# crowsonkb/k-diffusion

Measured on NVIDIA H100. Metric: images/sec (256x256, Heun 50-step), higher is better.
Workload: dtype bf16

## Files before the change

k-diffusion_b200/csrc/tc_common.cuh:

```cuda
#pragma once
#include <cuda.h>

#include "common.cuh"

namespace kdb {
namespace tc {

__device__ __forceinline__ uint32_t smem_u32(const void* p) { return (uint32_t)__cvta_generic_to_shared(p); }

__device__ __forceinline__ void pdl_wait() { asm volatile("griddepcontrol.wait;" ::: "memory"); }
__device__ __forceinline__ void pdl_launch_dependents() { asm volatile("griddepcontrol.launch_dependents;" ::: "memory"); }

__device__ __forceinline__ void mbar_init(uint64_t* bar, uint32_t count) {
  asm volatile("mbarrier.init.shared::cta.b64 [%0], %1;" ::"r"(smem_u32(bar)), "r"(count));
}
__device__ __forceinline__ void fence_barrier_init() { asm volatile("fence.mbarrier_init.release.cluster;" ::: "memory"); }
__device__ __forceinline__ void fence_proxy_async() { asm volatile("fence.proxy.async.shared::cta;" ::: "memory"); }

__device__ __forceinline__ void mbar_arrive_expect_tx(uint64_t* bar, uint32_t bytes) {
  asm volatile("mbarrier.arrive.expect_tx.shared::cta.b64 _, [%0], %1;" ::"r"(smem_u32(bar)), "r"(bytes) : "memory");
}
__device__ __forceinline__ void mbar_arrive(uint64_t* bar) {
  asm volatile("mbarrier.arrive.shared::cta.b64 _, [%0];" ::"r"(smem_u32(bar)) : "memory");
}
__device__ __forceinline__ bool mbar_try_wait(uint64_t* bar, uint32_t parity) {
  uint32_t ok;
  asm volatile(
      "{\n\t.reg .pred p;\n\t"
      "mbarrier.try_wait.parity.shared::cta.b64 p, [%1], %2, %3;\n\t"
      "selp.u32 %0, 1, 0, p;\n\t}"
      : "=r"(ok)
      : "r"(smem_u32(bar)), "r"(parity), "r"(200000u)
      : "memory");
  return ok != 0;
}
__device__ __forceinline__ uint64_t globaltimer_ns() {
  uint64_t t;
  asm volatile("mov.u64 %0, %%globaltimer;" : "=l"(t));
  return t;
}
__device__ __forceinline__ void mbar_wait(uint64_t* bar, uint32_t parity) {
  if (mbar_try_wait(bar, parity)) return;
  const uint64_t t0 = globaltimer_ns();
  uint32_t spins = 0;
  while (!mbar_try_wait(bar, parity)) {
    if ((++spins & 63u) == 0 && globaltimer_ns() - t0 > 2000000000ull) {
      printf("libkdb200: mbarrier wait timed out (block %d,%d,%d thread %d parity %u)\n", blockIdx.x, blockIdx.y, blockIdx.z, threadIdx.x, parity);
      __trap();
    }
  }
}

__device__ __forceinline__ void mbar_wait_nocall(uint64_t* bar, uint32_t parity) {
  if (mbar_try_wait(bar, parity)) return;
  const uint64_t t0 = globaltimer_ns();
  uint32_t spins = 0;
  while (!mbar_try_wait(bar, parity))
    if ((++spins & 63u) == 0 && globaltimer_ns() - t0 > 2000000000ull) __trap();
}

__device__ __forceinline__ void tma_prefetch_desc(const CUtensorMap* m) {
  asm volatile("prefetch.tensormap [%0];" ::"l"(reinterpret_cast<uint64_t>(m)) : "memory");
}
__device__ __forceinline__ void tma_load_2d(void* smem_dst, const CUtensorMap* map, uint64_t* bar, int c0, int c1) {
  asm volatile("cp.async.bulk.tensor.2d.shared::cluster.global.mbarrier::complete_tx::bytes [%0], [%1, {%3, %4}], [%2];" ::"r"(
                   smem_u32(smem_dst)),
               "l"(reinterpret_cast<uint64_t>(map)), "r"(smem_u32(bar)), "r"(c0), "r"(c1)
               : "memory");
}
__device__ __forceinline__ void tma_load_3d(void* smem_dst, const CUtensorMap* map, uint64_t* bar, int c0, int c1, int c2) {
  asm volatile("cp.async.bulk.tensor.3d.shared::cluster.global.mbarrier::complete_tx::bytes [%0], [%1, {%3, %4, %5}], [%2];" ::"r"(
                   smem_u32(smem_dst)),
               "l"(reinterpret_cast<uint64_t>(map)), "r"(smem_u32(bar)), "r"(c0), "r"(c1), "r"(c2)
               : "memory");
}
__device__ __forceinline__ void tma_load_4d(void* smem_dst, const CUtensorMap* map, uint64_t* bar, int c0, int c1, int c2, int c3) {
  asm volatile("cp.async.bulk.tensor.4d.shared::cluster.global.mbarrier::complete_tx::bytes [%0], [%1, {%3, %4, %5, %6}], [%2];" ::"r"(
                   smem_u32(smem_dst)),
               "l"(reinterpret_cast<uint64_t>(map)), "r"(smem_u32(bar)), "r"(c0), "r"(c1), "r"(c2), "r"(c3)
               : "memory");
}

__device__ __forceinline__ void tma_load_5d(void* smem_dst, const CUtensorMap* map, uint64_t* bar, int c0, int c1, int c2, int c3, int c4) {
  asm volatile("cp.async.bulk.tensor.5d.shared::cluster.global.mbarrier::complete_tx::bytes [%0], [%1, {%3, %4, %5, %6, %7}], [%2];" ::"r"(
                   smem_u32(smem_dst)),
               "l"(reinterpret_cast<uint64_t>(map)), "r"(smem_u32(bar)), "r"(c0), "r"(c1), "r"(c2), "r"(c3), "r"(c4)
               : "memory");
}
__device__ __forceinline__ void tma_store_4d(const CUtensorMap* map, const void* smem_src, int c0, int c1, int c2, int c3) {
  asm volatile("cp.async.bulk.tensor.4d.global.shared::cta.bulk_group [%0, {%2, %3, %4, %5}], [%1];" ::"l"(reinterpret_cast<uint64_t>(map)),
               "r"(smem_u32(smem_src)), "r"(c0), "r"(c1), "r"(c2), "r"(c3)
               : "memory");
}
__device__ __forceinline__ void tma_store_3d(const CUtensorMap* map, const void* smem_src, int c0, int c1, int c2) {
  asm volatile("cp.async.bulk.tensor.3d.global.shared::cta.bulk_group [%0, {%2, %3, %4}], [%1];" ::"l"(reinterpret_cast<uint64_t>(map)),
               "r"(smem_u32(smem_src)), "r"(c0), "r"(c1), "r"(c2)
               : "memory");
}
__device__ __forceinline__ void tma_store_2d(const CUtensorMap* map, const void* smem_src, int c0, int c1) {
  asm volatile("cp.async.bulk.tensor.2d.global.shared::cta.bulk_group [%0, {%2, %3}], [%1];" ::"l"(reinterpret_cast<uint64_t>(map)),
               "r"(smem_u32(smem_src)), "r"(c0), "r"(c1)
               : "memory");
}
__device__ __forceinline__ void tma_store_commit() { asm volatile("cp.async.bulk.commit_group;" ::: "memory"); }
__device__ __forceinline__ void tma_store_wait_read() { asm volatile("cp.async.bulk.wait_group.read 0;" ::: "memory"); }
__device__ __forceinline__ void named_barrier_sync(int id, int threads) { asm volatile("bar.sync %0, %1;" ::"r"(id), "r"(threads) : "memory"); }
__device__ __forceinline__ void named_barrier_arrive(int id, int threads) { asm volatile("bar.arrive %0, %1;" ::"r"(id), "r"(threads) : "memory"); }

template <uint32_t R> __device__ __forceinline__ void setmaxnreg_dec() { asm volatile("setmaxnreg.dec.sync.aligned.u32 %0;" ::"n"(R)); }
template <uint32_t R> __device__ __forceinline__ void setmaxnreg_inc() { asm volatile("setmaxnreg.inc.sync.aligned.u32 %0;" ::"n"(R)); }

__device__ __forceinline__ uint32_t sw128_offset(int row, int chunk16) {
  return (uint32_t)((row >> 3) * 1024 + (row & 7) * 128 + ((chunk16 ^ (row & 7)) << 4));
}

__device__ __forceinline__ void wg_fence() { asm volatile("wgmma.fence.sync.aligned;" ::: "memory"); }
__device__ __forceinline__ void wg_commit() { asm volatile("wgmma.commit_group.sync.aligned;" ::: "memory"); }
template <int N>
__device__ __forceinline__ void wg_wait() { asm volatile("wgmma.wait_group.sync.aligned %0;" ::"n"(N) : "memory"); }
template <int R>
__device__ __forceinline__ void wg_fence_acc(float (&d)[R]) {
#pragma unroll
  for (int i = 0; i < R; ++i) asm volatile("" : "+f"(d[i])::"memory");
}
template <int R>
__device__ __forceinline__ void wg_fence_acc(uint32_t (&d)[R]) {
#pragma unroll
  for (int i = 0; i < R; ++i) asm volatile("" : "+r"(d[i])::"memory");
}

__device__ __forceinline__ void wgmma_128(float (&d)[64], uint64_t adesc, uint64_t bdesc, uint32_t accumulate) {
  asm volatile(
      "{\n\t.reg .pred p;\n\t"
      "setp.ne.b32 p, %66, 0;\n\t"
      "wgmma.mma_async.sync.aligned.m64n128k16.f32.bf16.bf16 "
      "{%0, %1, %2, %3, %4, %5, %6, %7, %8, %9, %10, %11, %12, %13, %14, %15, %16, %17, %18, %19, %20, %21, %22, %23, %24, %25, %26, %27, %28, %29, %30, %31, %32, %33, %34, %35, %36, %37, %38, %39, %40, %41, %42, %43, %44, %45, %46, %47, %48, %49, %50, %51, %52, %53, %54, %55, %56, %57, %58, %59, %60, %61, %62, %63}, %64, %65, p, 1, 1, 0, 0;\n\t}"
      : "+f"(d[0]), "+f"(d[1]), "+f"(d[2]), "+f"(d[3]), "+f"(d[4]), "+f"(d[5]), "+f"(d[6]), "+f"(d[7]), "+f"(d[8]), "+f"(d[9]), "+f"(d[10]), "+f"(d[11]), "+f"(d[12]), "+f"(d[13]), "+f"(d[14]), "+f"(d[15]), "+f"(d[16]), "+f"(d[17]), "+f"(d[18]), "+f"(d[19]), "+f"(d[20]), "+f"(d[21]), "+f"(d[22]), "+f"(d[23]), "+f"(d[24]), "+f"(d[25]), "+f"(d[26]), "+f"(d[27]), "+f"(d[28]), "+f"(d[29]), "+f"(d[30]), "+f"(d[31]), "+f"(d[32]), "+f"(d[33]), "+f"(d[34]), "+f"(d[35]), "+f"(d[36]), "+f"(d[37]), "+f"(d[38]), "+f"(d[39]), "+f"(d[40]), "+f"(d[41]), "+f"(d[42]), "+f"(d[43]), "+f"(d[44]), "+f"(d[45]), "+f"(d[46]), "+f"(d[47]), "+f"(d[48]), "+f"(d[49]), "+f"(d[50]), "+f"(d[51]), "+f"(d[52]), "+f"(d[53]), "+f"(d[54]), "+f"(d[55]), "+f"(d[56]), "+f"(d[57]), "+f"(d[58]), "+f"(d[59]), "+f"(d[60]), "+f"(d[61]), "+f"(d[62]), "+f"(d[63])
      : "l"(adesc), "l"(bdesc), "r"(accumulate));
}
template <int TB>
__device__ __forceinline__ void wgmma_64(float (&d)[32], uint64_t adesc, uint64_t bdesc, uint32_t accumulate) {
  asm volatile(
      "{\n\t.reg .pred p;\n\t"
      "setp.ne.b32 p, %34, 0;\n\t"
      "wgmma.mma_async.sync.aligned.m64n64k16.f32.bf16.bf16 "
      "{%0, %1, %2, %3, %4, %5, %6, %7, %8, %9, %10, %11, %12, %13, %14, %15, %16, %17, %18, %19, %20, %21, %22, %23, %24, %25, %26, %27, %28, %29, %30, %31}, %32, %33, p, 1, 1, 0, %35;\n\t}"
      : "+f"(d[0]), "+f"(d[1]), "+f"(d[2]), "+f"(d[3]), "+f"(d[4]), "+f"(d[5]), "+f"(d[6]), "+f"(d[7]), "+f"(d[8]), "+f"(d[9]), "+f"(d[10]), "+f"(d[11]), "+f"(d[12]), "+f"(d[13]), "+f"(d[14]), "+f"(d[15]), "+f"(d[16]), "+f"(d[17]), "+f"(d[18]), "+f"(d[19]), "+f"(d[20]), "+f"(d[21]), "+f"(d[22]), "+f"(d[23]), "+f"(d[24]), "+f"(d[25]), "+f"(d[26]), "+f"(d[27]), "+f"(d[28]), "+f"(d[29]), "+f"(d[30]), "+f"(d[31])
      : "l"(adesc), "l"(bdesc), "r"(accumulate), "n"(TB));
}
__device__ __forceinline__ void wgmma_128_rs(float (&d)[64], const uint32_t (&a)[4], uint64_t bdesc, uint32_t accumulate) {
  asm volatile(
      "{\n\t.reg .pred p;\n\t"
      "setp.ne.b32 p, %69, 0;\n\t"
      "wgmma.mma_async.sync.aligned.m64n128k16.f32.bf16.bf16 "
      "{%0, %1, %2, %3, %4, %5, %6, %7, %8, %9, %10, %11, %12, %13, %14, %15, %16, %17, %18, %19, %20, %21, %22, %23, %24, %25, %26, %27, %28, %29, %30, %31, %32, %33, %34, %35, %36, %37, %38, %39, %40, %41, %42, %43, %44, %45, %46, %47, %48, %49, %50, %51, %52, %53, %54, %55, %56, %57, %58, %59, %60, %61, %62, %63}, {%64, %65, %66, %67}, %68, p, 1, 1, 0;\n\t}"
      : "+f"(d[0]), "+f"(d[1]), "+f"(d[2]), "+f"(d[3]), "+f"(d[4]), "+f"(d[5]), "+f"(d[6]), "+f"(d[7]), "+f"(d[8]), "+f"(d[9]), "+f"(d[10]), "+f"(d[11]), "+f"(d[12]), "+f"(d[13]), "+f"(d[14]), "+f"(d[15]), "+f"(d[16]), "+f"(d[17]), "+f"(d[18]), "+f"(d[19]), "+f"(d[20]), "+f"(d[21]), "+f"(d[22]), "+f"(d[23]), "+f"(d[24]), "+f"(d[25]), "+f"(d[26]), "+f"(d[27]), "+f"(d[28]), "+f"(d[29]), "+f"(d[30]), "+f"(d[31]), "+f"(d[32]), "+f"(d[33]), "+f"(d[34]), "+f"(d[35]), "+f"(d[36]), "+f"(d[37]), "+f"(d[38]), "+f"(d[39]), "+f"(d[40]), "+f"(d[41]), "+f"(d[42]), "+f"(d[43]), "+f"(d[44]), "+f"(d[45]), "+f"(d[46]), "+f"(d[47]), "+f"(d[48]), "+f"(d[49]), "+f"(d[50]), "+f"(d[51]), "+f"(d[52]), "+f"(d[53]), "+f"(d[54]), "+f"(d[55]), "+f"(d[56]), "+f"(d[57]), "+f"(d[58]), "+f"(d[59]), "+f"(d[60]), "+f"(d[61]), "+f"(d[62]), "+f"(d[63])
      : "r"(a[0]), "r"(a[1]), "r"(a[2]), "r"(a[3]), "l"(bdesc), "r"(accumulate));
}

template <int TB>
__device__ __forceinline__ void wgmma_64_rs(float (&d)[32], const uint32_t (&a)[4], uint64_t bdesc, uint32_t accumulate) {
  asm volatile(
      "{\n\t.reg .pred p;\n\t"
      "setp.ne.b32 p, %37, 0;\n\t"
      "wgmma.mma_async.sync.aligned.m64n64k16.f32.bf16.bf16 "
      "{%0, %1, %2, %3, %4, %5, %6, %7, %8, %9, %10, %11, %12, %13, %14, %15, %16, %17, %18, %19, %20, %21, %22, %23, %24, %25, %26, %27, %28, %29, %30, %31}, {%32, %33, %34, %35}, %36, p, 1, 1, %38;\n\t}"
      : "+f"(d[0]), "+f"(d[1]), "+f"(d[2]), "+f"(d[3]), "+f"(d[4]), "+f"(d[5]), "+f"(d[6]), "+f"(d[7]), "+f"(d[8]), "+f"(d[9]), "+f"(d[10]), "+f"(d[11]), "+f"(d[12]), "+f"(d[13]), "+f"(d[14]), "+f"(d[15]), "+f"(d[16]), "+f"(d[17]), "+f"(d[18]), "+f"(d[19]), "+f"(d[20]), "+f"(d[21]), "+f"(d[22]), "+f"(d[23]), "+f"(d[24]), "+f"(d[25]), "+f"(d[26]), "+f"(d[27]), "+f"(d[28]), "+f"(d[29]), "+f"(d[30]), "+f"(d[31])
      : "r"(a[0]), "r"(a[1]), "r"(a[2]), "r"(a[3]), "l"(bdesc), "r"(accumulate), "n"(TB));
}

template <int R>
__device__ __forceinline__ void acc_store(float* s, int ld, int row0, const float (&d)[R]) {
  const int t = threadIdx.x & 127;
  const int r = row0 + 16 * (t >> 5) + ((t & 31) >> 2), c = 2 * (t & 3);
#pragma unroll
  for (int j = 0; j < R / 4; ++j) {
    *reinterpret_cast<float2*>(s + (size_t)r * ld + 8 * j + c) = make_float2(d[4 * j], d[4 * j + 1]);
    *reinterpret_cast<float2*>(s + (size_t)(r + 8) * ld + 8 * j + c) = make_float2(d[4 * j + 2], d[4 * j + 3]);
  }
}
__device__ __forceinline__ void acc_ld32(const float* s, int ld, int row, int col0, float (&v)[32]) {
  const float4* src = reinterpret_cast<const float4*>(s + (size_t)row * ld + col0);
#pragma unroll
  for (int i = 0; i < 8; ++i) {
    const float4 q = src[i];
    v[4 * i] = q.x;
// ... 100 lines not shown
```

k-diffusion_b200/csrc/tc_kernels.cu:

```cuda
#include "tc_common.cuh"
#include "tc_kernels.cuh"

namespace kdb {

typedef CUresult (*EncodeTiledFn)(CUtensorMap*, CUtensorMapDataType, cuuint32_t, void*, const cuuint64_t*, const cuuint64_t*,
                                  const cuuint32_t*, const cuuint32_t*, CUtensorMapInterleave, CUtensorMapSwizzle,
                                  CUtensorMapL2promotion, CUtensorMapFloatOOBfill);

static EncodeTiledFn encode_fn() {
  static EncodeTiledFn fn = [] {
    void* p = nullptr;
    cudaDriverEntryPointQueryResult q;
    if (cudaGetDriverEntryPoint("cuTensorMapEncodeTiled", &p, cudaEnableDefault, &q) != cudaSuccess) p = nullptr;
    return reinterpret_cast<EncodeTiledFn>(p);
  }();
  return fn;
}

int make_tmap_bf16(CUtensorMap* out, const void* base, int rank, const uint64_t* dims, const uint64_t* strides_bytes, const uint32_t* box) {
  EncodeTiledFn fn = encode_fn();
  KDB_REQUIRE(fn != nullptr, KDB_ERR_UNSUPPORTED, "cuTensorMapEncodeTiled not available from this driver");
  cuuint64_t gd[5];
  cuuint64_t gs[5];
  cuuint32_t bx[5], es[5];
  for (int i = 0; i < rank; ++i) {
    gd[i] = dims[i];
    bx[i] = box[i];
    es[i] = 1;
    if (i > 0) gs[i - 1] = strides_bytes[i - 1];
  }
  CUresult r = fn(out, CU_TENSOR_MAP_DATA_TYPE_BFLOAT16, (cuuint32_t)rank, const_cast<void*>(base), gd, gs, bx, es,
                  CU_TENSOR_MAP_INTERLEAVE_NONE, CU_TENSOR_MAP_SWIZZLE_128B, CU_TENSOR_MAP_L2_PROMOTION_L2_256B,
                  CU_TENSOR_MAP_FLOAT_OOB_FILL_NONE);
  KDB_REQUIRE(r == CUDA_SUCCESS, KDB_ERR_BAD_ARG, "cuTensorMapEncodeTiled failed with CUresult %d (rank %d, dim0 %llu, box0 %u)", (int)r,
              rank, (unsigned long long)dims[0], box[0]);
  return 0;
}

bool pdl_enabled() {
  static const bool enabled = [] {
    const char* e = getenv("KDB200_NO_PDL");
    return !(e != nullptr && e[0] == '1');
  }();
  return enabled;
}

namespace {

constexpr int BM = 128, BK = 64;
constexpr int A_STAGE_BYTES = BM * BK * 2;
constexpr int SUB_TILE_BYTES = BM * 128;
constexpr int GEMM_THREADS = 384;
constexpr int GEMM_RING_BYTES = 96 * 1024;

enum TcEpi { TCE_STORE = 0, TCE_RESID = 1, TCE_GEGLU = 2, TCE_SPLIT = 3, TCE_QKV = 4, TCE_PATCHOUT = 5 };

struct TcParams {
  bf16* out;
  const bf16* resid;
  const float* fac;
  int64_t M;
  int N, K;
  int hc, wc, Cf;
  const float2* rope;
  const float* qk_scale;
  int C, nh, T;
  float* fout;
  const float* x_in;
  const float* sigma;
  float sd;
  int H, Wimg, th, tw;
  const float* ss_in;
  float* ss_out;
  int a_merge, mwc, mC;
  int box_w, box_h;
};

__device__ __forceinline__ float bf16_round(float v) { return __bfloat162float(__float2bfloat16_rn(v)); }

int tmap_2d(CUtensorMap* t, const void* base, uint64_t inner, uint64_t outer, uint32_t box_inner, uint32_t box_outer) {
  const uint64_t dims[2] = {inner, outer};
  const uint64_t strides[1] = {inner * 2};
  const uint32_t box[2] = {box_inner, box_outer};
  return make_tmap_bf16(t, base, 2, dims, strides, box);
}

int tmap_quad(CUtensorMap* t, const void* base, int C, int wc, uint64_t bhc, int box_w, int box_h) {
  const uint64_t dims[5] = {(uint64_t)C, 2, (uint64_t)wc, 2, bhc};
  const uint64_t strides[4] = {(uint64_t)C * 2, (uint64_t)C * 4, (uint64_t)wc * C * 4, (uint64_t)wc * C * 8};
  const uint32_t box[5] = {64, 1, (uint32_t)box_w, 1, (uint32_t)box_h};
  return make_tmap_bf16(t, base, 5, dims, strides, box);
}

bool quad_box(int wc, int* box_w, int* box_h) {
  if (wc >= BM) {
    if (wc % BM != 0) return false;
    *box_w = BM;
    *box_h = 1;
    return true;
  }
  if (BM % wc != 0) return false;
  *box_w = wc;
  *box_h = BM / wc;
  return true;
}

template <int BN, int EPI> constexpr int out_bytes() {
  return EPI == TCE_GEGLU ? SUB_TILE_BYTES : (EPI == TCE_SPLIT || EPI == TCE_PATCHOUT) ? 0 : (BN / 64) * SUB_TILE_BYTES;
}
template <int BN, int EPI> constexpr size_t gemm_smem() { return 1024 + GEMM_RING_BYTES + BM * BN * 4 + 2 * out_bytes<BN, EPI>() + 128; }

template <int BN> __device__ __forceinline__ int stage_off(int row, int chunk) { return row * BN + ((chunk ^ (row & 7)) << 2); }
template <int BN>
__device__ __forceinline__ void stage_store(float* s, int row0, const float (&d)[BN / 2]) {
  const int t = threadIdx.x & 127;
  const int r = row0 + 16 * (t >> 5) + ((t & 31) >> 2), c = 2 * (t & 3);
#pragma unroll
  for (int j = 0; j < BN / 8; ++j) {
    *reinterpret_cast<float2*>(s + stage_off<BN>(r, 2 * j + (c >> 2)) + (c & 3)) = make_float2(d[4 * j], d[4 * j + 1]);
    *reinterpret_cast<float2*>(s + stage_off<BN>(r + 8, 2 * j + (c >> 2)) + (c & 3)) = make_float2(d[4 * j + 2], d[4 * j + 3]);
  }
}
template <int BN>
__device__ __forceinline__ void stage_ld32(const float* s, int row, int col0, float (&v)[32]) {
#pragma unroll
  for (int i = 0; i < 8; ++i) {
    const float4 q = *reinterpret_cast<const float4*>(s + stage_off<BN>(row, (col0 >> 2) + i));
    v[4 * i] = q.x;
    v[4 * i + 1] = q.y;
    v[4 * i + 2] = q.z;
    v[4 * i + 3] = q.w;
  }
}

template <int BN, int EPI>
__global__ void __launch_bounds__(GEMM_THREADS, 1) gemm_wg_kernel(const __grid_constant__ CUtensorMap tma, const __grid_constant__ CUtensorMap tmb,
                                                                  const __grid_constant__ CUtensorMap tmc, const __grid_constant__ CUtensorMap tmr,
                                                                  const TcParams p) {
  KDB_PDL_TRIGGER();
  extern __shared__ uint8_t smem_raw[];
  constexpr int B_STAGE_BYTES = BN * BK * 2;
  constexpr int STAGE_BYTES = A_STAGE_BYTES + B_STAGE_BYTES;
  constexpr int STAGES = GEMM_RING_BYTES / STAGE_BYTES;
  constexpr int NSUB = BN / 64;
  constexpr bool RES = EPI == TCE_RESID;
  uint8_t* base = reinterpret_cast<uint8_t*>((reinterpret_cast<uintptr_t>(smem_raw) + 1023) & ~(uintptr_t)1023);
  float* sAcc = reinterpret_cast<float*>(base + GEMM_RING_BYTES);
  uint64_t* full = reinterpret_cast<uint64_t*>(base + GEMM_RING_BYTES + BM * BN * 4 + 2 * out_bytes<BN, EPI>());
  uint64_t* empty = full + STAGES;
  uint64_t* resid_full = empty + STAGES;

  const int warp = threadIdx.x >> 5, lane = threadIdx.x & 31;
  const int nkb = p.K / BK;
  const int n_tiles = p.N / BN;
  const int tiles = (int)((p.M + BM - 1) / BM) * n_tiles;
  const int n_local = (int)blockIdx.x < tiles ? (tiles - 1 - (int)blockIdx.x) / (int)gridDim.x + 1 : 0;

  if (threadIdx.x == 0) {
    tc::tma_prefetch_desc(&tma);
    tc::tma_prefetch_desc(&tmb);
    for (int s = 0; s < STAGES; ++s) {
      tc::mbar_init(&full[s], 1);
      tc::mbar_init(&empty[s], 4);
    }
    tc::mbar_init(&resid_full[0], 1);
    tc::mbar_init(&resid_full[1], 1);
    tc::fence_barrier_init();
  }
  __syncthreads();
  tc::pdl_wait();

  if (warp >= 8) {
    tc::setmaxnreg_dec<40>();
    if (warp == 8 && tc::elect_one()) {
      int it = 0;
      for (int i = 0; i < n_local; ++i) {
        const int t = (int)blockIdx.x + i * (int)gridDim.x;
        const int64_t m0 = (int64_t)(t / n_tiles) * BM;
        const int n0 = (t % n_tiles) * BN;
        for (int kb = 0; kb < nkb; ++kb, ++it) {
          const int s = it % STAGES;
          tc::mbar_wait_nocall(&empty[s], ((uint32_t)(it / STAGES) & 1u) ^ 1u);
          tc::mbar_arrive_expect_tx(&full[s], STAGE_BYTES);
          uint8_t* a = base + (size_t)s * STAGE_BYTES;
          if (p.a_merge) {
            const int qd = (kb * BK) / p.mC, e0 = kb * BK - qd * p.mC;
            tc::tma_load_5d(a, &tma, &full[s], e0, qd & 1, p.box_h == 1 ? (int)(m0 % p.mwc) : 0, qd >> 1, (int)(m0 / p.mwc));
          } else {
            tc::tma_load_2d(a, &tma, &full[s], kb * BK, (int)m0);
          }
          tc::tma_load_2d(a + A_STAGE_BYTES, &tmb, &full[s], kb * BK, n0);
        }
      }
    }
    return;
  }
  tc::setmaxnreg_inc<232>();

  const int wg = warp >> 2;
  const int row = threadIdx.x & 127;
  uint8_t* sC = base + GEMM_RING_BYTES + BM * BN * 4 + wg * out_bytes<BN, EPI>();
  const int ebar = 1 + wg;
  for (int i = wg; i < n_local; i += 2) {
    const int t = (int)blockIdx.x + i * (int)gridDim.x;
    const int64_t m0 = (int64_t)(t / n_tiles) * BM;
    const int n0 = (t % n_tiles) * BN;
    if constexpr (RES) {
      if (row == 0) {
        tc::mbar_arrive_expect_tx(&resid_full[wg], NSUB * SUB_TILE_BYTES);
#pragma unroll
        for (int g = 0; g < NSUB; ++g) tc::tma_load_2d(sC + g * SUB_TILE_BYTES, &tmr, &resid_full[wg], n0 + g * 64, (int)m0);
      }
    }

    float acc0[BN / 2], acc1[BN / 2];
#pragma unroll
    for (int k = 0; k < BN / 2; ++k) acc0[k] = acc1[k] = 0.f;
    if (i > 0) tc::named_barrier_sync(3 + wg, 256);
    const int it0 = i * nkb;
    for (int kb = 0; kb < nkb; ++kb) {
      const int s = (it0 + kb) % STAGES;
      tc::mbar_wait_nocall(&full[s], (uint32_t)((it0 + kb) / STAGES) & 1u);
      const uint32_t a_addr = tc::smem_u32(base + (size_t)s * STAGE_BYTES);
      const uint64_t ad0 = tc::smem_desc_k_sw128(a_addr), ad1 = tc::smem_desc_k_sw128(a_addr + 8 * 1024);
      const uint64_t bd = tc::smem_desc_k_sw128(a_addr + A_STAGE_BYTES);
      tc::wg_fence_acc(acc0);
      tc::wg_fence_acc(acc1);
      tc::wg_fence();
#pragma unroll
      for (int k = 0; k < BK / 16; ++k) {
        if constexpr (BN == 128) {
          tc::wgmma_128(acc0, ad0 + 2ull * k, bd + 2ull * k, 1u);
          tc::wgmma_128(acc1, ad1 + 2ull * k, bd + 2ull * k, 1u);
        } else {
          tc::wgmma_64<0>(acc0, ad0 + 2ull * k, bd + 2ull * k, 1u);
          tc::wgmma_64<0>(acc1, ad1 + 2ull * k, bd + 2ull * k, 1u);
        }
      }
      tc::wg_commit();
      tc::wg_wait<1>();
      tc::wg_fence_acc(acc0);
      tc::wg_fence_acc(acc1);
      if (kb > 0 && lane == 0) tc::mbar_arrive(&empty[(it0 + kb - 1) % STAGES]);
    }
    if (i + 1 < n_local) tc::named_barrier_arrive(3 + (wg ^ 1), 256);
    tc::wg_wait<0>();
    tc::wg_fence_acc(acc0);
    tc::wg_fence_acc(acc1);
    if (lane == 0) tc::mbar_arrive(&empty[(it0 + nkb - 1) % STAGES]);
    if (i > 0) tc::named_barrier_sync(5 + wg, 256);
    stage_store<BN>(sAcc, 0, acc0);
    stage_store<BN>(sAcc, 64, acc1);
    tc::named_barrier_sync(ebar, 128);
    const bool pass_acc = i + 1 < n_local;

    const int64_t m = m0 + row;
    float rstd = 1.f;
    if (p.ss_in != nullptr) {
      const float4* sp = reinterpret_cast<const float4*>(p.ss_in + (m < p.M ? m : 0) * SS_PARTS);
      rstd = rsqrtf(tc::rowss_sum(__ldg(sp), __ldg(sp + 1), p.K >> 7) / (float)p.K + 1e-6f);
    }
    if constexpr (EPI == TCE_PATCHOUT) {
      float v[64];
      {
        float t0[32], t1[32];
        stage_ld32<BN>(sAcc, row, 0, t0);
        stage_ld32<BN>(sAcc, row, 32, t1);
#pragma unroll
        for (int k = 0; k < 32; ++k) { v[k] = t0[k]; v[32 + k] = t1[k]; }
      }
      if (pass_acc) tc::named_barrier_arrive(5 + (wg ^ 1), 256);
      if (m < p.M) {
        if (p.ss_in != nullptr) {
#pragma unroll
          for (int k = 0; k < 48; ++k) v[k] *= rstd;
        }
        const int per = p.th * p.tw;
        const int b = (int)(m / per);
        const int r = (int)(m - (int64_t)b * per);
        const int ty = r / p.tw, tx = r - ty * p.tw;
        float c_skip = 0.f, c_out = 1.f, c_in;
        if (p.sd > 0.f) karras_scalings(__ldg(p.sigma + b), p.sd, c_skip, c_out, c_in);
#pragma unroll
        for (int c = 0; c < 3; ++c)
#pragma unroll
          for (int nh = 0; nh < 4; ++nh) {
            const int64_t o = (((int64_t)b * 3 + c) * p.H + (ty * 4 + nh)) * p.Wimg + tx * 4;
            float4 y = make_float4(bf16_round(v[(nh * 4 + 0) * 3 + c]), bf16_round(v[(nh * 4 + 1) * 3 + c]), bf16_round(v[(nh * 4 + 2) * 3 + c]),
                                   bf16_round(v[(nh * 4 + 3) * 3 + c]));
            if (p.sd > 0.f) {
              const float4 xi = __ldg(reinterpret_cast<const float4*>(p.x_in + o));
              y = make_float4(y.x * c_out + xi.x * c_skip, y.y * c_out + xi.y * c_skip, y.z * c_out + xi.z * c_skip, y.w * c_out + xi.w * c_skip);
            }
            *reinterpret_cast<float4*>(p.fout + o) = y;
          }
      }
    } else if constexpr (EPI == TCE_SPLIT) {
      const bool live = m < p.M;
      const float facv = __ldg(p.fac);
      float ss = 0.f;
      int64_t fine = 0;
#pragma unroll 1
      for (int c = 0; c < BN / 32; ++c) {
        float v[32];
        stage_ld32<BN>(sAcc, row, c * 32, v);
        if (c == BN / 32 - 1 && pass_acc) tc::named_barrier_arrive(5 + (wg ^ 1), 256);
        if (!live) continue;
        const int n = n0 + c * 32;
        const int64_t b = m / ((int64_t)p.hc * p.wc);
        const int r = (int)(m - b * p.hc * p.wc);
        const int hy = r / p.wc, wx = r - hy * p.wc;
        const int qd = n / p.Cf, e = n - qd * p.Cf;
        fine = (b * (2 * p.hc) + (2 * hy + (qd >> 1))) * (2 * p.wc) + (2 * wx + (qd & 1));
        const int64_t off = fine * p.Cf + e;
        const uint4* sk = reinterpret_cast<const uint4*>(p.resid + off);
        uint4* dst = reinterpret_cast<uint4*>(p.out + off);
#pragma unroll
        for (int j = 0; j < 4; ++j) {
          const uint4 r4 = sk[j];
          const uint32_t rw[4] = {r4.x, r4.y, r4.z, r4.w};
          uint32_t ow[4];
#pragma unroll
          for (int q = 0; q < 4; ++q) {
            const float lo = __uint_as_float(rw[q] << 16), hi = __uint_as_float(rw[q] & 0xffff0000u);
            const float e0 = v[j * 8 + q * 2], e1 = v[j * 8 + q * 2 + 1];
            const float d0 = e0 - lo, d1 = e1 - hi;
            const float o0 = (facv < 0.5f) ? fmaf(facv, d0, lo) : e0 - d0 * (1.f - facv);
            const float o1 = (facv < 0.5f) ? fmaf(facv, d1, hi) : e1 - d1 * (1.f - facv);
            ss = fmaf(o0, o0, fmaf(o1, o1, ss));
            ow[q] = tc::pack_bf16x2(o0, o1);
          }
          dst[j] = make_uint4(ow[0], ow[1], ow[2], ow[3]);
        }
      }
      if (p.ss_out != nullptr && live) p.ss_out[fine * SS_PARTS + ((n0 % p.Cf) >> 7)] = ss;
    } else {
      if constexpr (RES) tc::mbar_wait_nocall(&resid_full[wg], (uint32_t)(i >> 1) & 1u);
      float ss_acc[4] = {0.f, 0.f, 0.f, 0.f};
#pragma unroll 1
      for (int g = 0; g < NSUB; ++g) {
        float v[64];
        {
          float t0[32], t1[32];
          stage_ld32<BN>(sAcc, row, g * 64, t0);
          stage_ld32<BN>(sAcc, row, g * 64 + 32, t1);
#pragma unroll
          for (int k = 0; k < 32; ++k) { v[k] = t0[k]; v[32 + k] = t1[k]; }
        }
        if (g == NSUB - 1 && pass_acc) tc::named_barrier_arrive(5 + (wg ^ 1), 256);
        if (EPI != TCE_GEGLU && p.ss_in != nullptr) {
          bool apply = true;
          if constexpr (EPI == TCE_QKV) apply = (n0 + g * 64) >= 2 * p.C;
          if (apply) {
#pragma unroll
            for (int k = 0; k < 64; ++k) v[k] *= rstd;
          }
        }
        if constexpr (EPI == TCE_GEGLU) {
          const tc::f32x2 r2 = tc::pk2(rstd, rstd), rh = tc::pk2(0.5f * rstd, 0.5f * rstd);
#pragma unroll
          for (int gg = 0; gg < 4; ++gg) {
            uint32_t o[4];
#pragma unroll
            for (int j = 0; j < 4; ++j) {
              tc::f32x2 val = tc::pk2(v[gg * 16 + 2 * j], v[gg * 16 + 2 * j + 1]);
              tc::f32x2 gate = tc::pk2(v[gg * 16 + 8 + 2 * j], v[gg * 16 + 8 + 2 * j + 1]);
              val = tc::mul2(val, rh);
              if (p.ss_in != nullptr) gate = tc::mul2(gate, r2);
              float o0, o1;
              tc::upk2(tc::geglu2(val, gate), o0, o1);
              o[j] = tc::pack_bf16x2(o0, o1);
            }
            *reinterpret_cast<uint4*>(sC + tc::sw128_offset(row, g * 4 + gg)) = make_uint4(o[0], o[1], o[2], o[3]);
          }
        } else {
          uint8_t* cg = sC + g * SUB_TILE_BYTES;
          if constexpr (RES) {
#pragma unroll
            for (int j = 0; j < 8; ++j) {
              const uint4 r4 = *reinterpret_cast<const uint4*>(cg + tc::sw128_offset(row, j));
              const uint32_t rw[4] = {r4.x, r4.y, r4.z, r4.w};
#pragma unroll
              for (int q = 0; q < 4; ++q) {
                v[j * 8 + q * 2] += __uint_as_float(rw[q] << 16);
                v[j * 8 + q * 2 + 1] += __uint_as_float(rw[q] & 0xffff0000u);
              }
            }
          }
          if constexpr (RES || EPI == TCE_STORE) {
            if (p.ss_out != nullptr) {
#pragma unroll
              for (int k = 0; k < 64; k += 4) {
                ss_acc[0] = fmaf(v[k], v[k], ss_acc[0]);
                ss_acc[1] = fmaf(v[k + 1], v[k + 1], ss_acc[1]);
                ss_acc[2] = fmaf(v[k + 2], v[k + 2], ss_acc[2]);
                ss_acc[3] = fmaf(v[k + 3], v[k + 3], ss_acc[3]);
              }
            }
          }
          if constexpr (EPI == TCE_QKV) {
            const int n = n0 + g * 64;
            const int t3 = n / p.C, head = (n - t3 * p.C) >> 6;
            if (t3 < 2) {
              const int64_t tok = (m < p.M ? m : 0) % p.T;
              const float4* tb = reinterpret_cast<const float4*>(p.rope) + (int64_t)head * 8 * p.T + tok;
              tc::f32x2 P[32];
#pragma unroll
              for (int k = 0; k < 32; ++k) P[k] = tc::pk2(v[2 * k], v[2 * k + 1]);
              tc::f32x2 q0 = tc::mul2(P[0], P[0]), q1 = tc::mul2(P[1], P[1]), q2 = tc::mul2(P[2], P[2]), q3 = tc::mul2(P[3], P[3]);
#pragma unroll
              for (int k = 4; k < 32; k += 4) {
                q0 = tc::fma2(P[k], P[k], q0);
                q1 = tc::fma2(P[k + 1], P[k + 1], q1);
                q2 = tc::fma2(P[k + 2], P[k + 2], q2);
                q3 = tc::fma2(P[k + 3], P[k + 3], q3);
              }
              const float sc = sqrtf(__ldg(p.qk_scale + head)) * rsqrtf(((q0.x + q0.y) + (q1.x + q1.y)) + ((q2.x + q2.y) + (q3.x + q3.y)) + 1e-6f);
              const tc::f32x2 sc2 = tc::pk2(sc, sc);
#pragma unroll
              for (int k = 0; k < 8; ++k) {
                const float4 cs = __ldg(tb + (int64_t)k * p.T);
                const tc::f32x2 C = tc::pk2(cs.x, cs.y), S = tc::pk2(cs.z, cs.w);
                const tc::f32x2 X1 = P[k], X2 = P[8 + k];
                P[k] = tc::mul2(tc::fma2(X2, tc::neg2(S), tc::mul2(X1, C)), sc2);
                P[8 + k] = tc::mul2(tc::fma2(X1, S, tc::mul2(X2, C)), sc2);
              }
#pragma unroll
              for (int k = 16; k < 32; ++k) P[k] = tc::mul2(P[k], sc2);
#pragma unroll
              for (int k = 0; k < 32; ++k) tc::upk2(P[k], v[2 * k], v[2 * k + 1]);
            }
          }
#pragma unroll
          for (int j = 0; j < 8; ++j)
            *reinterpret_cast<uint4*>(cg + tc::sw128_offset(row, j)) =
                make_uint4(tc::pack_bf16x2(v[j * 8 + 0], v[j * 8 + 1]), tc::pack_bf16x2(v[j * 8 + 2], v[j * 8 + 3]),
                           tc::pack_bf16x2(v[j * 8 + 4], v[j * 8 + 5]), tc::pack_bf16x2(v[j * 8 + 6], v[j * 8 + 7]));
        }
      }
      if constexpr (RES || EPI == TCE_STORE) {
        if (p.ss_out != nullptr && m < p.M) p.ss_out[m * SS_PARTS + (n0 >> 7)] = (ss_acc[0] + ss_acc[1]) + (ss_acc[2] + ss_acc[3]);
      }
      tc::fence_proxy_async();
      tc::named_barrier_sync(ebar, 128);
      if (row == 0) {
        if constexpr (EPI == TCE_GEGLU) {
          tc::tma_store_2d(&tmc, sC, n0 / 2, (int)m0);
        } else {
#pragma unroll
          for (int g = 0; g < NSUB; ++g) tc::tma_store_2d(&tmc, sC + g * SUB_TILE_BYTES, n0 + g * 64, (int)m0);
        }
        tc::tma_store_commit();
        tc::tma_store_wait_read();
      }
    }
  }
}


#include "tc_ffn_fused.cuh"
#include "tc_attn_block.cuh"

template <int BN, int EPI>
int launch_tc(const bf16* A, const bf16* W, const TcParams& p, cudaStream_t st) {
  CUtensorMap ta, tb, tcm, tr;
  int rc;
  if (p.a_merge) {
    if ((rc = tmap_quad(&ta, A, p.mC, p.mwc, (uint64_t)p.M / p.mwc, p.box_w, p.box_h))) return rc;
  } else {
    if ((rc = tmap_2d(&ta, A, (uint64_t)p.K, (uint64_t)p.M, BK, BM))) return rc;
  }
  if ((rc = tmap_2d(&tb, W, (uint64_t)p.K, (uint64_t)p.N, BK, BN))) return rc;
  const uint64_t n_out = EPI == TCE_GEGLU ? (uint64_t)p.N / 2 : (uint64_t)p.N;
  if (EPI != TCE_SPLIT && EPI != TCE_PATCHOUT) {
    if ((rc = tmap_2d(&tcm, p.out, n_out, (uint64_t)p.M, 64, BM))) return rc;
  } else {
    tcm = ta;
  }
  if (EPI == TCE_RESID) {
    if ((rc = tmap_2d(&tr, p.resid, (uint64_t)p.N, (uint64_t)p.M, 64, BM))) return rc;
  } else {
    tr = ta;
  }
  constexpr size_t smem = gemm_smem<BN, EPI>();
  static_assert(smem <= 227 * 1024, "GEMM shared memory exceeds the 227 KiB opt-in limit");
  static bool attr_set = false;
  if (!attr_set) {
    KDB_CUDA(cudaFuncSetAttribute(gemm_wg_kernel<BN, EPI>, cudaFuncAttributeMaxDynamicSharedMemorySize, (int)smem));
    attr_set = true;
  }
  const int64_t tiles = ceil_div(p.M, BM) * (p.N / BN);
  KDB_CUDA(launch_pdl(gemm_wg_kernel<BN, EPI>, dim3((unsigned)(tiles < num_sms() ? tiles : num_sms())), dim3(GEMM_THREADS), smem, st, ta, tb, tcm,
                      tr, p));
  KDB_LAUNCH_CHECK(EPI == TCE_PATCHOUT ? F_PATCH_OUT : F_GEMM_TC, st);
  return 0;
}

template <int EPI>
int dispatch_bn(const bf16* A, const bf16* W, const TcParams& p, cudaStream_t st) {
  if (p.N % 128 == 0) return launch_tc<128, EPI>(A, W, p, st);
  return launch_tc<64, EPI>(A, W, p, st);
}

bool shape_ok(int64_t M, int N, int K) {
  return M > 0 && M < (65535LL * BM) && N >= 64 && N % 64 == 0 && K >= 64 && K % 64 == 0;
}

}

namespace {
struct PatchInParams {
  const float* x;
  const float* sigma;
  float sd;
  int64_t M;
  int H, Wimg, th, tw, N;
  float* ss_out;
};

constexpr int PATCH_IN_THREADS = 160;
constexpr int PATCH_IN_LD = 132;
constexpr size_t PATCH_IN_SMEM = 1024 + 2 * A_STAGE_BYTES + (size_t)BM * PATCH_IN_LD * 4 + 2 * SUB_TILE_BYTES + 64;

__global__ void __launch_bounds__(PATCH_IN_THREADS) patch_in_tc_kernel(const __grid_constant__ CUtensorMap tmw, const __grid_constant__ CUtensorMap tmc,
                                                                   const PatchInParams p) {
  KDB_PDL_TRIGGER();
  extern __shared__ uint8_t smem_raw[];
  constexpr int LD = PATCH_IN_LD;
  uint8_t* base = reinterpret_cast<uint8_t*>((reinterpret_cast<uintptr_t>(smem_raw) + 1023) & ~(uintptr_t)1023);
  uint8_t* sA = base;
  uint8_t* sW = base + A_STAGE_BYTES;
  uint8_t* sC = sW + A_STAGE_BYTES;
  float* sAcc = reinterpret_cast<float*>(sC + 2 * SUB_TILE_BYTES);
  uint64_t* w_full = reinterpret_cast<uint64_t*>(sAcc + BM * LD);

  const int warp = threadIdx.x >> 5;
  const int64_t m0 = (int64_t)blockIdx.x * BM;
  const int n0 = blockIdx.y * 128;
  if (threadIdx.x == 0) {
    tc::tma_prefetch_desc(&tmw);
    tc::tma_prefetch_desc(&tmc);
    tc::mbar_init(w_full, 1);
    tc::fence_barrier_init();
  }
  __syncthreads();

  if (warp == 4) {
    if (tc::elect_one()) {
      tc::mbar_arrive_expect_tx(w_full, A_STAGE_BYTES);
      tc::tma_load_2d(sW, &tmw, w_full, 0, n0);
    }
    return;
  }
  const int row = threadIdx.x;
  const int64_t m = m0 + row;
  uint4 chunk[6];
  if (m < p.M) {
    const int per = p.th * p.tw;
    const int b = (int)(m / per);
    const int r = (int)(m - (int64_t)b * per);
    const int ty = r / p.tw, tx = r - ty * p.tw;
    float c_in = 1.f;
    if (p.sd > 0.f) {
      const float sg = __ldg(p.sigma + b);
      c_in = rsqrtf(fmaf(sg, sg, p.sd * p.sd));
// ... 70 lines not shown
  tc::fence_proxy_async();
  tc::named_barrier_sync(1, 128);
  if (threadIdx.x == 0) {
    tc::tma_store_2d(&tmc, sC, n0, (int)m0);
    tc::tma_store_2d(&tmc, sC + SUB_TILE_BYTES, n0 + 64, (int)m0);
    tc::tma_store_commit();
    tc::tma_store_wait_read();
  }
}

__global__ void __launch_bounds__(256) patch_in_weight_kernel(const float* __restrict__ W, bf16* __restrict__ out, int N) {
  for (int i = blockIdx.x * 256 + threadIdx.x; i < N * 64; i += gridDim.x * 256) {
    const int n = i >> 6, k = i & 63;
    float v = 0.f;
    if (k < 48) {
      const int c = k >> 4, nh = (k >> 2) & 3, nw = k & 3;
      v = W[(int64_t)n * 48 + (nh * 4 + nw) * 3 + c];
    }
    out[i] = __float2bfloat16(v);
  }
}

}

static bool g_tc_disabled = [] {
  const char* e = getenv("KDB200_DISABLE_TC");
  return e != nullptr && e[0] == '1';
}();

bool tc_gemm_supported(int64_t M, int N, int K, const GemmEpi& epi) {
  if (g_tc_disabled || !shape_ok(M, N, K)) return false;
  if (epi.ss_in != nullptr && (N % 128 != 0 || K % 128 != 0 || K > 128 * SS_PARTS || (epi.mode != EPI_STORE && epi.mode != EPI_QKV_ROPE) || epi.mC > 0))
    return false;
  if (epi.mC > 0) {
    int bw, bh;
    if (epi.mode != EPI_STORE || N % 128 != 0 || epi.mC % 64 != 0 || K != 4 * epi.mC || M % epi.mwc != 0 || !quad_box(epi.mwc, &bw, &bh)) return false;
  }
  if (epi.mode == EPI_SPLIT_LERP) return epi.C % 32 == 0 && N == 4 * epi.C;
  if (epi.mode == EPI_QKV_ROPE) return N == 3 * epi.C && epi.C % 64 == 0 && epi.nh * 64 == epi.C && epi.rope != nullptr;
  return epi.mode == EPI_STORE || epi.mode == EPI_RESID;
}

bool tc_gemm_emits_rowss(int64_t M, int N, int K, const GemmEpi& epi) {
  if (!tc_gemm_supported(M, N, K, epi)) return false;
  if (N % 128 != 0) return false;
  if (epi.mode == EPI_RESID || epi.mode == EPI_STORE) return N <= 128 * SS_PARTS;
  if (epi.mode == EPI_SPLIT_LERP) return epi.C % 128 == 0 && epi.C <= 128 * SS_PARTS;
  return false;
}

int launch_gemm_tc(const bf16* A, const bf16* W, bf16* C, int64_t M, int N, int K, const GemmEpi& epi, cudaStream_t st) {
  KDB_REQUIRE(shape_ok(M, N, K), KDB_ERR_BAD_SHAPE, "gemm_tc: unsupported shape M=%lld N=%d K=%d", (long long)M, N, K);
  KDB_REQUIRE((reinterpret_cast<uintptr_t>(A) & 15) == 0 && (reinterpret_cast<uintptr_t>(W) & 15) == 0 && (reinterpret_cast<uintptr_t>(C) & 15) == 0,
              KDB_ERR_BAD_ARG, "gemm_tc: operands must be 16-byte aligned");
  TcParams p{};
  p.out = C;
  p.M = M;
  p.N = N;
  p.K = K;
  p.ss_in = epi.ss_in;
  p.ss_out = epi.ss_out;
  KDB_REQUIRE(epi.ss_in == nullptr || tc_gemm_supported(M, N, K, epi), KDB_ERR_UNSUPPORTED, "gemm_tc: fused-norm geometry not supported");
  KDB_REQUIRE(epi.ss_out == nullptr || tc_gemm_emits_rowss(M, N, K, epi), KDB_ERR_UNSUPPORTED, "gemm_tc: this shape cannot emit row statistics");
  if (epi.mC > 0) {
    KDB_REQUIRE(tc_gemm_supported(M, N, K, epi), KDB_ERR_UNSUPPORTED, "gemm_tc: token-merge geometry not supported");
    p.a_merge = 1;
    p.mC = epi.mC;
    p.mwc = epi.mwc;
    quad_box(epi.mwc, &p.box_w, &p.box_h);
    return launch_tc<128, TCE_STORE>(A, W, p, st);
  }
  switch (epi.mode) {
    case EPI_STORE:
      return dispatch_bn<TCE_STORE>(A, W, p, st);
    case EPI_RESID:
      p.resid = static_cast<const bf16*>(epi.resid);
      return dispatch_bn<TCE_RESID>(A, W, p, st);
    case EPI_SPLIT_LERP:
      p.resid = static_cast<const bf16*>(epi.resid);
      p.fac = epi.fac;
      p.hc = epi.hc;
      p.wc = epi.wc;
      p.Cf = epi.C;
      return dispatch_bn<TCE_SPLIT>(A, W, p, st);
    case EPI_QKV_ROPE:
      p.rope = epi.rope;
      p.qk_scale = epi.qk_scale;
      p.C = epi.C;
      p.nh = epi.nh;
      p.T = epi.T_tokens;
      return dispatch_bn<TCE_QKV>(A, W, p, st);
    default:
      KDB_REQUIRE(false, KDB_ERR_BAD_ARG, "gemm_tc: bad epilogue");
  }
}

bool tc_patch_out_supported(int C0, int Cout, int ph, int pw, int Wimg) {
  return !g_tc_disabled && C0 % 64 == 0 && Cout == 3 && ph == 4 && pw == 4 && Wimg % 4 == 0;
}

int launch_patch_out_tc(const bf16* xn, const bf16* W_pad, const float* x_in, const float* sigma, float sigma_data, float* out, int B, int H,
                        int Wimg, int C0, cudaStream_t st, const float* ss_in) {
  KDB_REQUIRE(ss_in == nullptr || (C0 % 128 == 0 && C0 <= 128 * SS_PARTS), KDB_ERR_UNSUPPORTED, "patch_out_tc: fused norm needs C0 %% 128 == 0");
  KDB_REQUIRE((reinterpret_cast<uintptr_t>(out) & 15) == 0 && (sigma_data <= 0.f || (reinterpret_cast<uintptr_t>(x_in) & 15) == 0), KDB_ERR_BAD_ARG,
              "patch_out_tc: x and out must be 16-byte aligned (float4 epilogue)");
  TcParams p{};
  p.ss_in = ss_in;
  p.M = (int64_t)B * (H / 4) * (Wimg / 4);
  p.N = 64;
  p.K = C0;
  p.fout = out;
  p.x_in = x_in;
  p.sigma = sigma;
  p.sd = sigma_data;
  p.H = H;
  p.Wimg = Wimg;
  p.th = H / 4;
  p.tw = Wimg / 4;
  KDB_REQUIRE(shape_ok(p.M, 64, C0), KDB_ERR_BAD_SHAPE, "patch_out_tc: unsupported shape");
  return launch_tc<64, TCE_PATCHOUT>(xn, W_pad, p, st);
}

bool tc_patch_in_supported(int Cin, int ph, int pw, int C0, int Wimg) {
  return !g_tc_disabled && Cin == 3 && ph == 4 && pw == 4 && C0 % 128 == 0 && C0 <= 128 * SS_PARTS && Wimg % 4 == 0;
}

int prepare_patch_in_weight(const float* W, bf16* out, int C0, cudaStream_t st) {
  patch_in_weight_kernel<<<(unsigned)ceil_div((int64_t)C0 * 64, 256), 256, 0, st>>>(W, out, C0);
  KDB_LAUNCH_CHECK(F_CONVERT, st);
  return 0;
}

int launch_patch_in_tc(const float* x, const float* sigma, float sigma_data, const bf16* W_perm, bf16* out, int B, int H, int Wimg, int C0,
                       float* ss_out, cudaStream_t st) {
  PatchInParams p{};
  p.x = x;
  p.sigma = sigma;
  p.sd = sigma_data;
  p.H = H;
  p.Wimg = Wimg;
  p.th = H / 4;
  p.tw = Wimg / 4;
  p.M = (int64_t)B * p.th * p.tw;
  p.N = C0;
  p.ss_out = ss_out;
  KDB_REQUIRE((reinterpret_cast<uintptr_t>(x) & 15) == 0, KDB_ERR_BAD_ARG, "patch_in_tc: input must be 16-byte aligned");
  CUtensorMap tw, tcm;
  int rc;
  if ((rc = tmap_2d(&tw, W_perm, 64, (uint64_t)C0, 64, 128))) return rc;
  if ((rc = tmap_2d(&tcm, out, (uint64_t)C0, (uint64_t)p.M, 64, BM))) return rc;
  const size_t smem = PATCH_IN_SMEM;
  static bool attr_set = false;
  if (!attr_set) {
    KDB_CUDA(cudaFuncSetAttribute(patch_in_tc_kernel, cudaFuncAttributeMaxDynamicSharedMemorySize, (int)smem));
    attr_set = true;
  }
  patch_in_tc_kernel<<<dim3((unsigned)ceil_div(p.M, BM), (unsigned)(C0 / 128)), PATCH_IN_THREADS, smem, st>>>(tw, tcm, p);
  KDB_LAUNCH_CHECK(F_PATCH_IN, st);
  return 0;
}

bool tc_gemm_geglu_supported(int64_t M, int N2, int K, bool fused_norm) {
  if (fused_norm && (K % 128 != 0 || K > 128 * SS_PARTS)) return false;
  return !g_tc_disabled && shape_ok(M, N2, K) && N2 % 128 == 0;
}

// ... 95 lines not shown
```

Baseline: 125.5.

## Use TMA preload and TMA store for split-lerp GEMM epilogue

Adds a TCE_SPLIT_TMA epilogue variant for the token-split/lerp GEMM. It prefetches the skip/residual tile into shared memory with a 5D TMA load in the quad layout, does the lerp in swizzled smem, and writes the result back with 5D TMA stores. This replaces the per-thread scattered global loads and stores of the old split epilogue. It is dispatched only when C is a multiple of 64 and the tile fits a quad box; otherwise the old path is kept. It also adds unused multicast and cluster helpers.

```diff
diff --git a/k-diffusion_b200/csrc/tc_common.cuh b/k-diffusion_b200/csrc/tc_common.cuh
--- a/k-diffusion_b200/csrc/tc_common.cuh
+++ b/k-diffusion_b200/csrc/tc_common.cuh
@@ -87,6 +87,11 @@
                "l"(reinterpret_cast<uint64_t>(map)), "r"(smem_u32(bar)), "r"(c0), "r"(c1), "r"(c2), "r"(c3), "r"(c4)
                : "memory");
 }
+__device__ __forceinline__ void tma_store_5d(const CUtensorMap* map, const void* smem_src, int c0, int c1, int c2, int c3, int c4) {
+  asm volatile("cp.async.bulk.tensor.5d.global.shared::cta.bulk_group [%0, {%2, %3, %4, %5, %6}], [%1];" ::"l"(reinterpret_cast<uint64_t>(map)),
+               "r"(smem_u32(smem_src)), "r"(c0), "r"(c1), "r"(c2), "r"(c3), "r"(c4)
+               : "memory");
+}
 __device__ __forceinline__ void tma_store_4d(const CUtensorMap* map, const void* smem_src, int c0, int c1, int c2, int c3) {
   asm volatile("cp.async.bulk.tensor.4d.global.shared::cta.bulk_group [%0, {%2, %3, %4, %5}], [%1];" ::"l"(reinterpret_cast<uint64_t>(map)),
                "r"(smem_u32(smem_src)), "r"(c0), "r"(c1), "r"(c2), "r"(c3)
@@ -102,6 +107,31 @@
                "r"(smem_u32(smem_src)), "r"(c0), "r"(c1)
                : "memory");
 }
+__device__ __forceinline__ void tma_load_2d_mc(void* smem_dst, const CUtensorMap* map, uint64_t* bar, int c0, int c1, uint16_t cta_mask) {
+  asm volatile(
+      "cp.async.bulk.tensor.2d.shared::cluster.global.mbarrier::complete_tx::bytes.multicast::cluster [%0], [%1, {%3, %4}], [%2], %5;" ::"r"(
+          smem_u32(smem_dst)),
+      "l"(reinterpret_cast<uint64_t>(map)), "r"(smem_u32(bar)), "r"(c0), "r"(c1), "h"(cta_mask)
+      : "memory");
+}
+
+__device__ __forceinline__ uint32_t cluster_ctarank() {
+  uint32_t r;
+  asm volatile("mov.u32 %0, %%cluster_ctarank;" : "=r"(r));
+  return r;
+}
+__device__ __forceinline__ void cluster_sync() {
+  asm volatile("barrier.cluster.arrive.release.aligned;\n\tbarrier.cluster.wait.acquire.aligned;" ::: "memory");
+}
+__device__ __forceinline__ void mbar_arrive_cluster(uint64_t* bar, uint32_t cta) {
+  asm volatile(
+      "{\n\t.reg .b32 ra;\n\t"
+      "mapa.shared::cluster.u32 ra, %0, %1;\n\t"
+      "mbarrier.arrive.shared::cluster.b64 _, [ra];\n\t}" ::"r"(smem_u32(bar)),
+      "r"(cta)
+      : "memory");
+}
+
 __device__ __forceinline__ void tma_store_commit() { asm volatile("cp.async.bulk.commit_group;" ::: "memory"); }
 __device__ __forceinline__ void tma_store_wait_read() { asm volatile("cp.async.bulk.wait_group.read 0;" ::: "memory"); }
 __device__ __forceinline__ void named_barrier_sync(int id, int threads) { asm volatile("bar.sync %0, %1;" ::"r"(id), "r"(threads) : "memory"); }
diff --git a/k-diffusion_b200/csrc/tc_kernels.cu b/k-diffusion_b200/csrc/tc_kernels.cu
--- a/k-diffusion_b200/csrc/tc_kernels.cu
+++ b/k-diffusion_b200/csrc/tc_kernels.cu
@@ -53,7 +53,7 @@
 constexpr int GEMM_THREADS = 384;
 constexpr int GEMM_RING_BYTES = 96 * 1024;
 
-enum TcEpi { TCE_STORE = 0, TCE_RESID = 1, TCE_GEGLU = 2, TCE_SPLIT = 3, TCE_QKV = 4, TCE_PATCHOUT = 5 };
+enum TcEpi { TCE_STORE = 0, TCE_RESID = 1, TCE_GEGLU = 2, TCE_SPLIT = 3, TCE_QKV = 4, TCE_PATCHOUT = 5, TCE_SPLIT_TMA = 6 };
 
 struct TcParams {
   bf16* out;
@@ -144,6 +144,7 @@
   constexpr int STAGES = GEMM_RING_BYTES / STAGE_BYTES;
   constexpr int NSUB = BN / 64;
   constexpr bool RES = EPI == TCE_RESID;
+  constexpr bool PRELOAD = RES || EPI == TCE_SPLIT_TMA;
   uint8_t* base = reinterpret_cast<uint8_t*>((reinterpret_cast<uintptr_t>(smem_raw) + 1023) & ~(uintptr_t)1023);
   float* sAcc = reinterpret_cast<float*>(base + GEMM_RING_BYTES);
   uint64_t* full = reinterpret_cast<uint64_t*>(base + GEMM_RING_BYTES + BM * BN * 4 + 2 * out_bytes<BN, EPI>());
@@ -205,11 +206,19 @@
     const int t = (int)blockIdx.x + i * (int)gridDim.x;
     const int64_t m0 = (int64_t)(t / n_tiles) * BM;
     const int n0 = (t % n_tiles) * BN;
-    if constexpr (RES) {
+    if constexpr (PRELOAD) {
       if (row == 0) {
         tc::mbar_arrive_expect_tx(&resid_full[wg], NSUB * SUB_TILE_BYTES);
 #pragma unroll
-        for (int g = 0; g < NSUB; ++g) tc::tma_load_2d(sC + g * SUB_TILE_BYTES, &tmr, &resid_full[wg], n0 + g * 64, (int)m0);
+        for (int g = 0; g < NSUB; ++g) {
+          if constexpr (RES) {
+            tc::tma_load_2d(sC + g * SUB_TILE_BYTES, &tmr, &resid_full[wg], n0 + g * 64, (int)m0);
+          } else {
+            const int qd = (n0 + g * 64) / p.Cf, e0 = n0 + g * 64 - qd * p.Cf;
+            tc::tma_load_5d(sC + g * SUB_TILE_BYTES, &tmr, &resid_full[wg], e0, qd & 1, p.box_h == 1 ? (int)(m0 % p.wc) : 0, qd >> 1,
+                            (int)(m0 / p.wc));
+          }
+        }
       }
     }
 
@@ -334,6 +343,59 @@
         }
       }
       if (p.ss_out != nullptr && live) p.ss_out[fine * SS_PARTS + ((n0 % p.Cf) >> 7)] = ss;
+    } else if constexpr (EPI == TCE_SPLIT_TMA) {
+      const float facv = __ldg(p.fac);
+      float ss = 0.f;
+      tc::mbar_wait_nocall(&resid_full[wg], (uint32_t)(i >> 1) & 1u);
+#pragma unroll 1
+      for (int g = 0; g < NSUB; ++g) {
+        float v[64];
+        {
+          float t0[32], t1[32];
+          stage_ld32<BN>(sAcc, row, g * 64, t0);
+          stage_ld32<BN>(sAcc, row, g * 64 + 32, t1);
+#pragma unroll
+          for (int k = 0; k < 32; ++k) { v[k] = t0[k]; v[32 + k] = t1[k]; }
+        }
+        if (g == NSUB - 1 && pass_acc) tc::named_barrier_arrive(5 + (wg ^ 1), 256);
+        uint8_t* cg = sC + g * SUB_TILE_BYTES;
+#pragma unroll
+        for (int j = 0; j < 8; ++j) {
+          const uint4 r4 = *reinterpret_cast<const uint4*>(cg + tc::sw128_offset(row, j));
+          const uint32_t rw[4] = {r4.x, r4.y, r4.z, r4.w};
+          uint32_t ow[4];
+#pragma unroll
+          for (int q = 0; q < 4; ++q) {
+            const float lo = __uint_as_float(rw[q] << 16), hi = __uint_as_float(rw[q] & 0xffff0000u);
+            const float e0 = v[j * 8 + q * 2], e1 = v[j * 8 + q * 2 + 1];
+            const float d0 = e0 - lo, d1 = e1 - hi;
+            const float o0 = (facv < 0.5f) ? fmaf(facv, d0, lo) : e0 - d0 * (1.f - facv);
+            const float o1 = (facv < 0.5f) ? fmaf(facv, d1, hi) : e1 - d1 * (1.f - facv);
+            ss = fmaf(o0, o0, fmaf(o1, o1, ss));
+            ow[q] = tc::pack_bf16x2(o0, o1);
+          }
+          *reinterpret_cast<uint4*>(cg + tc::sw128_offset(row, j)) = make_uint4(ow[0], ow[1], ow[2], ow[3]);
+        }
+      }
+      if (p.ss_out != nullptr && m < p.M) {
+        const int64_t b = m / ((int64_t)p.hc * p.wc);
+        const int r = (int)(m - b * p.hc * p.wc);
+        const int hy = r / p.wc, wx = r - hy * p.wc;
+        const int qd = n0 / p.Cf;
+        const int64_t fine = (b * (2 * p.hc) + (2 * hy + (qd >> 1))) * (2 * p.wc) + (2 * wx + (qd & 1));
+        p.ss_out[fine * SS_PARTS + ((n0 % p.Cf) >> 7)] = ss;
+      }
+      tc::fence_proxy_async();
+      tc::named_barrier_sync(ebar, 128);
+      if (row == 0) {
+#pragma unroll
+        for (int g = 0; g < NSUB; ++g) {
+          const int qd = (n0 + g * 64) / p.Cf, e0 = n0 + g * 64 - qd * p.Cf;
+          tc::tma_store_5d(&tmc, sC + g * SUB_TILE_BYTES, e0, qd & 1, p.box_h == 1 ? (int)(m0 % p.wc) : 0, qd >> 1, (int)(m0 / p.wc));
+        }
+        tc::tma_store_commit();
+        tc::tma_store_wait_read();
+      }
     } else {
       if constexpr (RES) tc::mbar_wait_nocall(&resid_full[wg], (uint32_t)(i >> 1) & 1u);
       float ss_acc[4] = {0.f, 0.f, 0.f, 0.f};
@@ -472,15 +534,20 @@
   }
   if ((rc = tmap_2d(&tb, W, (uint64_t)p.K, (uint64_t)p.N, BK, BN))) return rc;
   const uint64_t n_out = EPI == TCE_GEGLU ? (uint64_t)p.N / 2 : (uint64_t)p.N;
-  if (EPI != TCE_SPLIT && EPI != TCE_PATCHOUT) {
-    if ((rc = tmap_2d(&tcm, p.out, n_out, (uint64_t)p.M, 64, BM))) return rc;
+  if (EPI == TCE_SPLIT_TMA) {
+    if ((rc = tmap_quad(&tcm, p.out, p.Cf, p.wc, (uint64_t)p.M / p.wc, p.box_w, p.box_h))) return rc;
+    if ((rc = tmap_quad(&tr, p.resid, p.Cf, p.wc, (uint64_t)p.M / p.wc, p.box_w, p.box_h))) return rc;
   } else {
-    tcm = ta;
-  }
-  if (EPI == TCE_RESID) {
-    if ((rc = tmap_2d(&tr, p.resid, (uint64_t)p.N, (uint64_t)p.M, 64, BM))) return rc;
-  } else {
-    tr = ta;
+    if (EPI != TCE_SPLIT && EPI != TCE_PATCHOUT) {
+      if ((rc = tmap_2d(&tcm, p.out, n_out, (uint64_t)p.M, 64, BM))) return rc;
+    } else {
+      tcm = ta;
+    }
+    if (EPI == TCE_RESID) {
+      if ((rc = tmap_2d(&tr, p.resid, (uint64_t)p.N, (uint64_t)p.M, 64, BM))) return rc;
+    } else {
+      tr = ta;
+    }
   }
   constexpr size_t smem = gemm_smem<BN, EPI>();
   static_assert(smem <= 227 * 1024, "GEMM shared memory exceeds the 227 KiB opt-in limit");
@@ -717,6 +784,7 @@
       p.hc = epi.hc;
       p.wc = epi.wc;
       p.Cf = epi.C;
+      if (epi.C % 64 == 0 && M % epi.wc == 0 && quad_box(epi.wc, &p.box_w, &p.box_h)) return dispatch_bn<TCE_SPLIT_TMA>(A, W, p, st);
       return dispatch_bn<TCE_SPLIT>(A, W, p, st);
     case EPI_QKV_ROPE:
       p.rope = epi.rope;
```

Result: faster. 128.6 (median of 6 runs) (+2.5%).
